# bbw7561135/Compton2d

Measured on AMD Instinct MI355X. Metric: photon-packet-steps/sec (whole node) at 1/2/4/8 GPUs; % HBM roofline, higher is better.
Workload: dtype f64

## Files before the change

compton2d_amd/csrc/c2d_device.hpp:

```cpp
#ifndef C2D_DEVICE_HPP
#define C2D_DEVICE_HPP

#include <stdint.h>
#include "../../include/compton2d.h"

namespace c2d {

#define C2D_IDX_BUCKETS 2048
struct Geo {
  double z[C2D_MAXZONE + 1];
  double r[C2D_MAXZONE + 1];
  double E_ph[C2D_N_VOL + 1];
  double E_field[C2D_NPHFIELD + 1];
  double hu[C2D_NPHOMAX + 2];
  double Elcmin[C2D_NPHLCMAX + 1];
  double Elcmax[C2D_NPHLCMAX + 1];
  double mu[C2D_NMUMAX + 1];
  int16_t eph_start[C2D_IDX_BUCKETS];
  int16_t efl_start[C2D_IDX_BUCKETS];
  int32_t eph_k0, efl_k0;
};
constexpr int GEO_DOUBLES = (int)(sizeof(Geo) / sizeof(double));

struct SpecDev {
// ... 40 lines not shown
  uint32_t sub;
};

struct PktSoA {
  double* rpre; double* zpre; double* wmu; double* phi; double* ew; double* xnu; double* dcen;
  uint32_t* jk;
  uint32_t* bins;
  uint32_t* ctr;
  uint32_t* sub;
  uint64_t* key;
};

struct TallyOff {
  int64_t edep, prdep, ecens, npcen, n_field, E_IC, nelectron, fout, edout;
  int64_t erlki, erlko, erlku, erlkl, Ed_in, counters;
};

#define C2D_EV_SHARDS 32
#ifndef C2D_TR_BLOCK
#define C2D_TR_BLOCK 256
#endif
#define C2D_EV_SHARD_STRIDE 16
#define C2D_EVQ_WORDS 8
#define C2D_EVQ_MAX 64
#define C2D_WORK_SHARDS 64

#ifndef C2D_COMTAB_N
#define C2D_COMTAB_N 2048
#endif
#define C2D_COMTAB_U0 (-27.631021115928547)
#define C2D_COMTAB_U1 (29.933606208922594)

__device__ __forceinline__ double c2d_tau_log_f32(double u) {
  const float v = (float)(1.0 - u);
  const float w = 1.0f - v;
  const bool lo = u < 0.5;
  const float lg = 0.69314718f * __builtin_amdgcn_logf(lo ? (float)u : w);
  const float r = (w == 1.0f) ? -v : lg * (v * __builtin_amdgcn_rcpf(1.0f - w));
  return (double)(lo ? lg : r);
}

enum : int32_t {
  ERR_CENSUS = 1, ERR_EVENT = 2, ERR_QUEUE = 4, ERR_SPEC = 8, ERR_NONFINITE = 16
};

#define C2D_GLOBAL __attribute__((address_space(1)))
template <class T>
__device__ __forceinline__ T gld(const T* p) { return *(const C2D_GLOBAL T*)p; }
template <class T>
__device__ __forceinline__ void gst(T* p, T v) { *(C2D_GLOBAL T*)p = v; }
__device__ __forceinline__ void cst2(c2d_d2* p, double a, double b) {
  const c2d_d2 v = {a, b};
  *(C2D_GLOBAL c2d_d2*)p = v;
}
__device__ __forceinline__ c2d_d2 cld2(const c2d_d2* p) { return *(const C2D_GLOBAL c2d_d2*)p; }
__device__ __forceinline__ void cst4(c2d_u4* p, uint32_t jk, uint32_t bins, uint64_t key) {
  const c2d_u4 v = {jk, bins, (uint32_t)key, (uint32_t)(key >> 32)};
  *(C2D_GLOBAL c2d_u4*)p = v;
}
__device__ __forceinline__ c2d_u4 cld4(const c2d_u4* p) { return *(const C2D_GLOBAL c2d_u4*)p; }
__device__ __forceinline__ uint64_t c2d_tg_key(c2d_u4 t) { return ((uint64_t)t.w << 32) | (uint64_t)t.z; }
__device__ __forceinline__ void cst2_nt(c2d_d2* p, double a, double b) {
  const c2d_d2 v = {a, b};
  __builtin_nontemporal_store(v, (C2D_GLOBAL c2d_d2*)p);
}
__device__ __forceinline__ c2d_d2 cld2_nt(const c2d_d2* p) {
  return __builtin_nontemporal_load((const C2D_GLOBAL c2d_d2*)p);
}
__device__ __forceinline__ void cst4_nt(c2d_u4* p, uint32_t jk, uint32_t bins, uint64_t key) {
  const c2d_u4 v = {jk, bins, (uint32_t)key, (uint32_t)(key >> 32)};
  __builtin_nontemporal_store(v, (C2D_GLOBAL c2d_u4*)p);
}
__device__ __forceinline__ c2d_u4 cld4_nt(const c2d_u4* p) {
  return __builtin_nontemporal_load((const C2D_GLOBAL c2d_u4*)p);
}
__device__ __forceinline__ uint32_t cens_bins(const c2d_u4* tg, int64_t s) {
  return gld(reinterpret_cast<const uint32_t*>(tg + s) + 1);
}
__device__ __forceinline__ void cens_set_bins(c2d_u4* tg, int64_t s, uint32_t b) {
  gst(reinterpret_cast<uint32_t*>(tg + s) + 1, b);
}
__device__ __forceinline__ void gadd(double* p, double v) {
  __hip_atomic_fetch_add((C2D_GLOBAL double*)p, v, __ATOMIC_RELAXED, __HIP_MEMORY_SCOPE_AGENT);
}

__device__ __forceinline__ void gor(int32_t* p, int32_t v) {
  __hip_atomic_fetch_or((C2D_GLOBAL int32_t*)p, v, __ATOMIC_RELAXED, __HIP_MEMORY_SCOPE_AGENT);
}

#ifndef C2D_NF_REPL
#define C2D_NF_REPL 8
#endif

#define C2D_CNT_PATHS_INT 10
#define C2D_CNT_DEAD_INT 12
#define C2D_CNT_CREUSE_INT 13
#define C2D_CNT_CLOST_INT 14

struct KParams {
  int32_t nz, nr, ncell, nphtotal, nph_lc, nmu;
  int32_t split1, split2, split3, spl3_trg, spec_switch;
  int32_t rank, world, ncycle, eps_linear;
  double time, dt, rmin, zmin, cdt;
  double cens_wlim;
  uint64_t step_key;
  const Geo* geo;
  const double* gnt;
  const double* kappa_cv;
  const double* kappa_s;
  const double* eps_tot;
  const double* eps_th;
  const double* f_nt;
  const double* Pnt;
  const double* n_e;
  const double* vfrac;
  const double* ewsv;
  const int64_t* vol_prefix;
  const int64_t* surf_prefix;
  const double* surf_ew;
  const double* surf_tbb;
  const int32_t* surf_spec;
  const double* tbbl;
  const SpecDev* spectra;
  int32_t n_spectra, nslot;
  const double* comtab;
  double comtab_du_inv;
  double egg_min;
  CensusSoA cin, cout;
  int64_t n_cin, cap_cout;
  uint32_t cens_chunk;
  unsigned long long* n_cout;
  const int32_t* clist;
  const int32_t* pool;
  const unsigned long long* pool_n;
  unsigned long long* pool_head;
  int32_t* out_list;
  unsigned long long* n_out;
  int32_t* relist;
  unsigned long long* n_relist;
  unsigned long long* relist_head;
  int64_t* cstate;
  double* ev;
  int64_t cap_ev;
  unsigned long long* n_ev_sh;
  int64_t cap_ev_sh;
  int64_t cap_q;
  PktSoA pk;
  int64_t cap_pk;
  int64_t n_cens_items, n_vol_items, n_surf_items;
  int64_t vol_cens_base;
  int64_t n_vol_global, n_surf_global;
  double* T;
  double* nf_rep;
  TallyOff off;
  unsigned long long* cnt;
  int32_t* err;
  int32_t lds_cells;
  int32_t evq_cap;
  unsigned long long* prof;
  const uint16_t* cdf_guide;
};
#define C2D_CDF_GUIDE 256

#define C2D_KN_CAP_DEFAULT 32
#define C2D_SC_K1_DEFAULT 16
struct GenArgs {
// ... 116 lines not shown
```

compton2d_amd/csrc/transport.hip:

```cpp
#include <hip/hip_runtime.h>

#ifndef C2D_FAST_MDIV
#define C2D_FAST_MDIV 1
#endif
#if defined(C2D_VARIANT) && C2D_VARIANT == 1 && C2D_FAST_MDIV
__device__ __forceinline__ double c2d_mdiv_rcp(double a, double b) {
  double y = __builtin_amdgcn_rcp(b);
  y = __builtin_fma(y, __builtin_fma(-b, y, 1.0), y);
  y = __builtin_fma(y, __builtin_fma(-b, y, 1.0), y);
  return a * y;
}
#define C2D_MDIV(a, b) c2d_mdiv_rcp((a), (b))
#endif
#ifndef C2D_FAST_FMA
#define C2D_FAST_FMA 0
#endif
#if defined(C2D_VARIANT) && C2D_VARIANT == 1 && C2D_FAST_FMA
#define C2D_MADD(a, b, c) __builtin_fma((a), (b), (c))
#endif

#include "c2d_device.hpp"
#include "c2d_math.h"
#include "c2d_rng.h"

// ... 617 lines not shown
  double gams = clampd(1.0 - (znue - znues) / (znu * znus), lim);
  for (;;) {
    if (++guard > 4 * MAX_REJECT) { CB_CNT(C2D_CNT_ABORTED); break; }
    wa = U(p);
    wb = 2.0 * U(p) - 1.0;
    swa = wa * wa + wb * wb;
    if (swa >= 1.0 || swa <= 1.0e-20) continue;
    break;
  }
  double cazs = clampd((wa * wa - wb * wb) / swa, lim);
  double wmus = p.wmu * gams +
                cazs * __builtin_sqrt((1.0 - gams * gams) * (1.0 - p.wmu * p.wmu + fuzz));
  wmus = clampd(wmus, lim);
  double xnus = znus * EMASSKEV;
  double cosdphi = clampd((gams - p.wmu * wmus) /
                              __builtin_sqrt((1.0 - p.wmu * p.wmu) * (1.0 - wmus * wmus)),
                          lim);
  double dphi = c2d_acos(cosdphi);
  double phis = p.phi + dphi;
  set_bins(p, bin_sp(g, P.nphtotal, xnus, 1.000001, 0.999999, 0), bin_lc(g, P.nph_lc, xnus),
           bin_mu(g, P.nmu, wmus));
  p.ew = p.ew * xnus / p.xnu;
  p.xnu = xnus;
  p.wmu = wmus;
  p.phi = phis;
  return st.i;
}

template <int TALLY = 1>
__device__ __forceinline__ int compb2d_w(const KParams& P, const Geo* g, double* nel, Pkt& p, bool run,
                                          int kn_cap) {
  KnState st;
  st.i = 0; st.j = 0; st.ctrA = 0;
  bool need = false;
  if (run) need = !kn_loop<TALLY>(P, nel, p, st, kn_cap < MAX_REJECT - 1 ? kn_cap : MAX_REJECT - 1);
  kn_coop<TALLY>(P, nel, p, st, need);
  int i_gam = 0;
  if (run) i_gam = compb2d_b<TALLY>(P, g, p, st);
  return i_gam;
}

__device__ __forceinline__ void push_event(const KParams& P0, double tb, const Pkt& p, LaneCnt& lc) {
  const KParams& P = cold(P0);
  const unsigned sh = blockIdx.x % C2D_EV_SHARDS;
  const unsigned long long slot = wave_reserve(P.n_ev_sh + sh * C2D_EV_SHARD_STRIDE);
  if (slot < (unsigned long long)P.cap_ev_sh) {
    double* e = P.ev + ((int64_t)sh * P.cap_ev_sh + (int64_t)slot) * C2D_EVENT_WORDS;
#if C2D_EV_NT
    EV_ST(e, tb); EV_ST(e + 1, p.xnu); EV_ST(e + 2, p.ew); EV_ST(e + 3, p.rpre); EV_ST(e + 4, p.zpre);
    EV_ST(e + 5, p.wmu); EV_ST(e + 6, p.phi);
#else
    gst(e, tb); gst(e + 1, p.xnu); gst(e + 2, p.ew); gst(e + 3, p.rpre); gst(e + 4, p.zpre);
    gst(e + 5, p.wmu); gst(e + 6, p.phi);
#endif
  } else {
    gor(P.err, ERR_EVENT);
  }
  LC_ADD(lc, C2D_CNT_EVENTS);
}

__device__ __forceinline__ void escape_tally(const KParams& P0, const Tal& T, const Pkt& p) {
  const KParams& P = cold(P0);
  const int32_t jgpsp = JGPSP(p), jgplc = JGPLC(p), jgpmu = JGPMU(p);
  if (jgplc > 0) atomicAdd(&T_EDOUT(P, T)[(jgpmu - 1) * C2D_NPHLCMAX + (jgplc - 1)], FDIV_POS(p.ew, P.dt));
  if (jgpsp > 0 && P.spec_switch == 0)
    atomicAdd(&T_FOUT(P, T)[(jgpmu - 1) * C2D_NPHOMAX + (jgpsp - 1)], p.ew);
}

C2D_COLD_FN int imcleak(const KParams& P0, const Tal& T, Pkt& p, LaneCnt& lc) {
  const KParams& P = cold(P0);
  if (p.kph == 0) {
    if (P.rmin > 1.0e-10) {
      atomicAdd(&T_ERLKI(P, T)[p.jph - 1], p.ew);
      LC_ADD(lc, C2D_CNT_ESCAPES);
      return 1;
    }
    p.phi = 1.0e-6;
    p.kph = 1;
    return 0;
  }
  LC_ADD(lc, C2D_CNT_ESCAPES);
  const double tb = P.time + P.dt - RAD_CP * p.dcen;
  if (p.jph <= 0) {
    if (P.tbbl[p.kph - 1] > 0.0) {
      gadd(&P.T[P.off.Ed_in + p.kph - 1], p.ew);
      atomicAdd(&T_ERLKL(P, T)[p.kph - 1], p.ew);
    }
    if (P.ncycle > 0) {
      push_event(P, tb, p, lc);
      escape_tally(P, T, p);
    }
    return 1;
  }
  if (p.jph != P.nz + 1) {
    atomicAdd(&T_ERLKO(P, T)[p.jph - 1], p.ew);
    if (P.ncycle > 0) {
      push_event(P, tb, p, lc);
      escape_tally(P, T, p);
    }
    return 1;
  }
  atomicAdd(&T_ERLKU(P, T)[p.kph - 1], p.ew);
  if (P.ncycle > 0 && p.wmu < F32(0.98)) {
    push_event(P, tb, p, lc);
    escape_tally(P, T, p);
  }
  return 1;
}

__device__ __forceinline__ int evq_offset(int evq_off) {
  return evq_off + __builtin_amdgcn_readfirstlane((int)((threadIdx.x >> 6) * C2D_EVQ_WORDS * C2D_EVQ_MAX));
}
__device__ __forceinline__ void evq_store(double* q, uint32_t i, const Pkt& p) {
  constexpr uint32_t cap = C2D_EVQ_MAX;
  q[i] = p.xnu;
  q[cap + i] = p.ew;
  q[2 * cap + i] = p.rpre;
  q[3 * cap + i] = p.zpre;
  q[4 * cap + i] = p.wmu;
#if C2D_TABLE_COMTOT
  q[5 * cap + i] = p.eta;
  const uint32_t sw = p.esw == -1 ? 0x80000000u : 0u;
#else
  q[5 * cap + i] = p.phi;
  const uint32_t sw = 0u;
#endif
  q[6 * cap + i] = p.dcen;
  const uint64_t tag = ((uint64_t)p.bins << 32) | (uint64_t)((uint32_t)p.kph | ((uint32_t)p.jph << 16) | sw);
  q[7 * cap + i] = __longlong_as_double((long long)tag);
}

__device__ __forceinline__ void evq_flush(const KParams& P0, const Tal& T, const double* q,
                                          uint32_t n, uint32_t lane, LaneCnt& lc) {
  constexpr uint32_t cap = C2D_EVQ_MAX;
  const KParams& P = cold(P0);
  if (lane >= n) return;
  Pkt p;
  p.xnu = q[lane];
  p.ew = q[cap + lane];
  p.rpre = q[2 * cap + lane];
  p.zpre = q[3 * cap + lane];
  p.wmu = q[4 * cap + lane];
  const double az = q[5 * cap + lane];
  p.dcen = q[6 * cap + lane];
  const uint64_t tag = (uint64_t)__double_as_longlong(q[7 * cap + lane]);
  p.bins = (uint32_t)(tag >> 32);
  p.kph = (int32_t)(tag & 0xffffu);
  p.jph = (int32_t)((tag >> 16) & 0x7fffu);
  LC_ADD(lc, C2D_CNT_ESCAPES);
  if (p.kph == 0) {
    atomicAdd(&T_ERLKI(P, T)[p.jph - 1], p.ew);
    return;
  }
  bool ev = P.ncycle > 0;
  if (p.jph <= 0) {
    if (P.tbbl[p.kph - 1] > 0.0) {
      gadd(&P.T[P.off.Ed_in + p.kph - 1], p.ew);
      atomicAdd(&T_ERLKL(P, T)[p.kph - 1], p.ew);
    }
  } else if (p.jph != P.nz + 1) {
    atomicAdd(&T_ERLKO(P, T)[p.jph - 1], p.ew);
  } else {
    atomicAdd(&T_ERLKU(P, T)[p.kph - 1], p.ew);
    ev = ev && p.wmu < F32(0.98);
  }
  if (!ev) return;
#if C2D_TABLE_COMTOT
  p.phi = c2d_acos(az);
  if (tag & 0x80000000ull) p.phi = 2.0 * PI_REF - p.phi;
#else
  p.phi = az;
#endif
  const double tb = P.time + P.dt - RAD_CP * p.dcen;
  push_event(P, tb, p, lc);
  escape_tally(P, T, p);
}

__shared__ unsigned long long c2d_cch_base[C2D_TR_BLOCK / 64];
__shared__ uint32_t c2d_cch_used[C2D_TR_BLOCK / 64];
__shared__ int32_t c2d_ct_idx[C2D_TR_BLOCK / 64][C2D_CT_TRACK];
__shared__ uint32_t c2d_ct_rem[C2D_TR_BLOCK / 64][C2D_CT_TRACK];
__shared__ int32_t c2d_fs[C2D_TR_BLOCK / 64][C2D_CT_STACK];
__shared__ uint32_t c2d_fs_n[C2D_TR_BLOCK / 64];
static_assert(C2D_WORK_CHUNK == C2D_CCHUNK, "a work chunk must cover exactly one census chunk");

C2D_COLD_FN unsigned long long census_new_chunk(const KParams& P0, int w) {
  const KParams& P = cold(P0);
  if (!P.clist)
    return __hip_atomic_fetch_add((C2D_GLOBAL unsigned long long*)P.n_cout, (unsigned long long)P.cens_chunk,
                                  __ATOMIC_RELAXED, __HIP_MEMORY_SCOPE_AGENT);
  int32_t id = -1;
  const uint32_t ns = c2d_fs_n[w];
  if (ns > 0) {
    id = c2d_fs[w][ns - 1];
    c2d_fs_n[w] = ns - 1;
  } else {
    if (__hip_atomic_load((C2D_GLOBAL unsigned long long*)P.n_relist, __ATOMIC_RELAXED,
                          __HIP_MEMORY_SCOPE_AGENT) > __hip_atomic_load((C2D_GLOBAL unsigned long long*)
                                                                          P.relist_head, __ATOMIC_RELAXED,
                                                                        __HIP_MEMORY_SCOPE_AGENT)) {
      const unsigned long long h = atomicAdd(P.relist_head, 1ull);
      if (h < gld(P.n_relist))
        id = __hip_atomic_load((C2D_GLOBAL int32_t*)(P.relist + h), __ATOMIC_RELAXED, __HIP_MEMORY_SCOPE_AGENT);
    }
    if (id < 0) {
      const unsigned long long h = atomicAdd(P.pool_head, 1ull);
      if (h < gld(P.pool_n)) id = gld(P.pool + h);
    }
  }
  if (id < 0) return (unsigned long long)P.cap_cout;
  gst(P.out_list + atomicAdd(P.n_out, 1ull), id);
  return (unsigned long long)id << C2D_CCHUNK_LOG;
}

__device__ __forceinline__ unsigned long long census_slot_chunk(const KParams& P0) {
  const KParams& P = cold(P0);
  const int w = (int)(threadIdx.x >> 6);
  const unsigned long long mask = __ballot(1);
  const uint32_t leader = (uint32_t)(__ffsll((long long)mask) - 1);
  const uint32_t lane = lane_id();
  const unsigned long long lt = (lane == 0) ? 0ull : (mask & ((~0ull) >> (64 - lane)));
  const uint32_t rank = (uint32_t)__popcll(lt), k = (uint32_t)__popcll(mask);
  const unsigned long long base = c2d_cch_base[w];
  const uint32_t used = c2d_cch_used[w];
  const uint32_t CENS_CHUNK = P.cens_chunk;
  const uint32_t rem = CENS_CHUNK - used;
  if (k <= rem) {
    if (lane == leader) c2d_cch_used[w] = used + k;
    return base + used + rank;
  }
  unsigned long long nb = 0;
  if (lane == leader) nb = census_new_chunk(P, w);
  const uint32_t lo = __builtin_amdgcn_readlane((uint32_t)nb, leader);
  const uint32_t hi = __builtin_amdgcn_readlane((uint32_t)(nb >> 32), leader);
  nb = ((unsigned long long)hi << 32) | lo;
  if (lane == leader) { c2d_cch_base[w] = nb; c2d_cch_used[w] = k - rem; }
  return rank < rem ? base + used + rank : nb + (rank - rem);
}

__device__ __forceinline__ void census_chunk_load(const KParams& P0, int w, uint32_t lane) {
  const KParams& P = cold(P0);
  if (lane != 0) return;
  c2d_cch_base[w] = 0ull;
  c2d_cch_used[w] = P.cens_chunk;
  c2d_fs_n[w] = 0u;
  for (int e = 0; e < C2D_CT_TRACK; e++) c2d_ct_idx[w][e] = -1;
  const int64_t ws = (int64_t)blockIdx.x * (C2D_TR_BLOCK / 64) + w;
  const int64_t base = gld(P.cstate + 2 * ws);
  if (base >= 0) {
    c2d_cch_base[w] = (unsigned long long)base;
    c2d_cch_used[w] = (uint32_t)gld(P.cstate + 2 * ws + 1);
  }
}

__device__ __forceinline__ void census_relist(const KParams& P, int32_t id) {
  const unsigned long long h = atomicAdd(P.n_relist, 1ull);
  __hip_atomic_store((C2D_GLOBAL int32_t*)(P.relist + h), id, __ATOMIC_RELAXED, __HIP_MEMORY_SCOPE_AGENT);
}

__device__ __forceinline__ void census_chunk_store(const KParams& P0, int w, uint32_t lane) {
  const KParams& P = cold(P0);
  if (lane != 0) return;
  if (P.clist)
    for (uint32_t i = 0; i < c2d_fs_n[w]; i++) census_relist(P, c2d_fs[w][i]);
  const uint32_t used = c2d_cch_used[w];
  const unsigned long long base = c2d_cch_base[w];
  const int64_t ws = (int64_t)blockIdx.x * (C2D_TR_BLOCK / 64) + w;
  const bool part = used < P.cens_chunk && base < (unsigned long long)P.cap_cout;
  gst(P.cstate + 2 * ws, part ? (int64_t)base : (int64_t)-1);
  gst(P.cstate + 2 * ws + 1, (int64_t)used);
}

__device__ __forceinline__ void census_track(int w, int32_t id, uint32_t n) {
#pragma unroll 1
  for (int k = 0; k < C2D_CT_TRACK; k++) {
    const int e = (id + k) & (C2D_CT_TRACK - 1);
    if (c2d_ct_idx[w][e] < 0) {
      c2d_ct_idx[w][e] = id;
      c2d_ct_rem[w][e] = n;
      return;
    }
  }
  atomicAdd(&c2d_cnt_lds[C2D_CNT_CLOST_INT], 1u);
}

C2D_COLD_FN void census_item_done(const KParams& P0, long long slot) {
  const KParams& P = cold(P0);
  const int w = (int)(threadIdx.x >> 6);
  const int32_t id = (int32_t)(slot >> C2D_CCHUNK_LOG);
  int e = id & (C2D_CT_TRACK - 1);
  if (c2d_ct_idx[w][e] != id) {
    int k = 1;
#pragma unroll 1
    for (; k < C2D_CT_TRACK; k++)
      if (c2d_ct_idx[w][(id + k) & (C2D_CT_TRACK - 1)] == id) break;
    if (k == C2D_CT_TRACK) return;
    e = (id + k) & (C2D_CT_TRACK - 1);
  }
  if (atomicSub(&c2d_ct_rem[w][e], 1u) != 1u) return;
  c2d_ct_idx[w][e] = -1;
  const uint32_t s = atomicAdd(&c2d_fs_n[w], 1u);
  if (s < C2D_CT_STACK) {
    c2d_fs[w][s] = id;
  } else {
    atomicSub(&c2d_fs_n[w], 1u);
    census_relist(P, id);
  }
  atomicAdd(&c2d_cnt_lds[C2D_CNT_CREUSE_INT], 1u);
}

C2D_COLD_FN void census_write(const KParams& P0, const Tal& T, const Pkt& p, LaneCnt& lc) {
  const KParams& P = cold(P0);
  const Geo* g = T.g;
  int cell = (p.jph - 1) * P.nr + (p.kph - 1);
  cell_add(P, T, TC_NPCEN, cell, 1.0);
  cell_add(P, T, TC_ECENS, cell, p.ew);
#if defined(C2D_ABLATE_NFIELD) && C2D_ABLATE_NFIELD == 1
  if (p.xnu < 0.0) {
#else
  int efl = 0;
  if (p.xnu > P.egg_min) {
#endif
    const int known = (p.ie >> 16) - 1;
    const int i = known >= 0 ? known : grid_lookup(g->E_field, C2D_NPHFIELD, g->efl_start, g->efl_k0, p.xnu);
    efl = i;
    const double v = FDIV_POS(6.25e8 * p.ew, p.xnu);
#if defined(C2D_ABLATE_NFIELD) && C2D_ABLATE_NFIELD == 2
    if (v == 1.25e300)
#endif
#if defined(C2D_ABLATE_NFIELD) && C2D_ABLATE_NFIELD == 3
    gst(&P.nf_rep[(int64_t)(blockIdx.x % C2D_NF_REPL) * P.ncell * C2D_NPHFIELD +
                  (int64_t)cell * C2D_NPHFIELD + (i - 1)], v);
    if (v == 1.25e300)
#endif
    gadd(&P.nf_rep[(int64_t)(blockIdx.x % C2D_NF_REPL) * P.ncell * C2D_NPHFIELD +
                   (int64_t)cell * C2D_NPHFIELD + (i - 1)], v);
  }
  const unsigned long long slot = census_slot_chunk(P);
  if (slot < (unsigned long long)P.cap_cout) {
// ... 86 lines not shown
  TP_POST = 5,
  TP_PTS = 6,
  TP_CWR = 7,
  TP_ITER = 8,
  TP_LANES = 9,
  TP_GOT_W = 10, TP_GOT_L = 11,
  TP_CENS_W = 12, TP_CENS_L = 13,
  TP_LEAK_W = 14, TP_LEAK_L = 15,
  TP_COLL_W = 16, TP_COLL_L = 17,
  TP_RST_W = 18, TP_RST_L = 19,
  TP_NWAVE = 20,
  TP_FLUSH = 21,
  TP_FLUSH_W = 22, TP_FLUSH_L = 23
};
enum : int { TP_CNT0 = TP_GOT_W, TP_CNT1 = TP_RST_L };
struct Prof {
#ifdef C2D_TR_PROF
  uint64_t acc[C2D_TR_PROF_WORDS];
  uint64_t t;
#endif
};
#ifdef C2D_TR_PROF
#define TP_MARK(pf, i) do { const uint64_t _n = clock64(); (pf).acc[i] += _n - (pf).t; (pf).t = _n; } while (0)
#define TP_COUNT(pf, iw, il) do {                                                         \
    const unsigned long long _m = __ballot(1);                                            \
    if (lane_id() == (uint32_t)(__ffsll((long long)_m) - 1)) {                            \
      (pf).acc[iw] += 1; (pf).acc[il] += __popcll(_m);                                    \
    }                                                                                     \
  } while (0)
#define TP_REPORT(pf, P, lane) do {                                                       \
    (pf).acc[TP_NWAVE] = 1;                                                               \
    for (int i = 0; i < C2D_TR_PROF_WORDS; i++)                                           \
      if ((pf).acc[i] && ((lane) == 0 || (i >= TP_CNT0 && i <= TP_CNT1)))                 \
        atomicAdd(&(P).prof[i], (unsigned long long)(pf).acc[i]);                         \
  } while (0)
#else
#define TP_MARK(pf, i) do { } while (0)
#define TP_COUNT(pf, iw, il) do { } while (0)
#endif

template <int V12>
__device__ __forceinline__ int flight(const KParams& P, const Tal& T, Pkt& p, ComCache& cc, LaneCnt& lc,
                                      Prof& pf) {
  const double lim8 = V12 ? 1.0 : 9.9999999e-1, lim9 = V12 ? 1.0 : 0.999999999;
  const Geo* g = T.g;
#if C2D_TABLE_COMTOT && C2D_EARLY_LOADS
  const int cell_e = (p.jph - 1) * P.nr + (p.kph - 1);
  const double* tb_e = P.comtab + (int64_t)cell_e * C2D_COMTAB_N + (p.tg > 0 ? p.tg - 1 : 0);
  const double ey0 = gld(tb_e), ey1 = gld(tb_e + 1), ey2 = gld(tb_e + 2), ey3 = gld(tb_e + 3);
  const double ene = gld(P.n_e + cell_e);
  const double ekap = gld((KAP(p) ? P.kappa_s : P.kappa_cv) + (int64_t)cell_e * C2D_N_VOL + ((p.ie & 0xffff) - 1));
#endif
  double colmfp = 0.0;
  if (p.mode != 0) colmfp = (V12 && p.nflight != 0) ? p.cmfp : -c2d_log(U(p));
  if (p.ew < 1.0e-40) return FL_END;
  if (++p.nflight > MAX_FLIGHTS) {
    LC_ADD(lc, C2D_CNT_ABORTED);
    return FL_END;
  }
  p.wmu = clampd(p.wmu, lim8);
  const int cell = (p.jph - 1) * P.nr + (p.kph - 1);
  double comac = 0.0;
  if (p.mode != 0) {
#if C2D_TABLE_COMTOT && C2D_EARLY_LOADS
    comac = (p.tg == 0) ? comtot_exact(P, cell, p.xnu)
                        : comtot_interp(ey0, ey1, ey2, ey3, ene, p.tt);
    (void)cc;
#elif C2D_TABLE_COMTOT
    comac = comtot_table(P, cell, p.xnu, p.tg, p.tt);
    (void)cc;
#else
    if (cc.cell0 == cell) {
      comac = cc.v0;
    } else if (cc.cell1 == cell) {
      comac = cc.v1;
    } else {
      comac = comtot_exact(P, cell, p.xnu);
      cc.cell1 = cc.cell0; cc.v1 = cc.v0;
      cc.cell0 = cell; cc.v0 = comac;
    }
#endif
  }
  const double sigsc = comac;
  const double rkm1 = (p.kph == 1) ? P.rmin : g->r[p.kph - 1];
  const double xqsqleft = rkm1 * rkm1;
  double dcol;
  if (p.mode != 0)
    dcol = colmfp / sigsc;
  else
    dcol = 100 * (g->r[P.nr] > g->z[P.nz] ? g->r[P.nr] : g->z[P.nz]);
  double trld;
  int ikind;
  if (p.dcen <= dcol) { trld = p.dcen; ikind = 2; }
  else { trld = dcol; ikind = 3; }
  lc.steps++;
#if C2D_TABLE_COMTOT
  double Eta = p.eta;
  const int eta_switch = p.esw;
#else
  double Eta = c2d_cos(p.phi);
  const int eta_switch = (p.phi <= PI_REF && p.phi >= 1.0e-10) ? 1 : -1;
#endif
  if (!V12) Eta = clampd(Eta, lim8);
  const double rpre = p.rpre, zpre = p.zpre, wmu = p.wmu;
  const double disp = Eta * rpre;
  const double psq = rpre * rpre * (1.0 - Eta * Eta);
  int kbnd, inout, knew, jnew;
  double rbnd, Zbnd;
  if (Eta < 0.0 && psq < xqsqleft) {
    kbnd = p.kph - 1;
    inout = -1;
    rbnd = rkm1;
  } else {
    kbnd = p.kph;
    inout = 1;
    rbnd = g->r[p.kph];
  }
  double dpbsq = rbnd * rbnd - psq;
  if (dpbsq < 1.0e-6) dpbsq = 1.0e-6;
  const double disbr = (double)inout * __builtin_sqrt(dpbsq) - disp;
  const double swmu = __builtin_sqrt(1.0 - wmu * wmu);
  double trldb = disbr / swmu;
  double fr = disbr;
  const double Zr = zpre + wmu * trldb;
  const double zlow = (p.jph == 1) ? P.zmin : g->z[p.jph - 1];
  const double zup = g->z[p.jph];
  if (Zr > zup || Zr < zlow) {
    Zbnd = (Zr > zup) ? zup : zlow;
    knew = p.kph;
    jnew = (Zr > zup) ? p.jph + 1 : p.jph - 1;
    const double f = (Zbnd - zpre) * swmu / wmu;
    fr = f;
    rbnd = __builtin_sqrt(rpre * rpre + f * f + 2.0 * rpre * f * Eta);
    trldb = __builtin_sqrt(f * f + (Zbnd - zpre) * (Zbnd - zpre));
  } else {
    knew = p.kph + inout;
    jnew = p.jph;
    rbnd = (kbnd > 0) ? g->r[kbnd] : P.rmin;
    Zbnd = Zr;
  }
  double rnew, znew;
  if (trldb < trld) {
    ikind = 1;
    trld = trldb;
    rnew = rbnd;
    znew = Zbnd;
  } else {
    jnew = p.jph;
    knew = p.kph;
    const double f = trld * swmu;
    fr = f;
    rnew = __builtin_sqrt(f * f + rpre * rpre + 2.0 * f * rpre * Eta);
    znew = zpre + trld * wmu;
  }
  TP_MARK(pf, TP_GEOM);
#if C2D_TABLE_COMTOT && C2D_EARLY_LOADS
  double sigabs = 1.0e-40 + 1.0 * ekap;
#else
  const double* kap = KAP(p) ? P.kappa_s : P.kappa_cv;
  double sigabs = 1.0e-40 + 1.0 * gld(kap + (int64_t)cell * C2D_N_VOL + ((p.ie & 0xffff) - 1));
#endif
  if (sigabs < 1.0e-40) sigabs = 1.0e-40;
  const double xabs = sigabs * trld;
  const double ewnew = (xabs < 100.0) ? p.ew * c2d_exp(-xabs) : 0.0;
  double deleabs = p.ew - ewnew;
  if (deleabs < 1.0e-50) deleabs = 1.0e-50;
  double wmustar;
  if (xabs <= 0.00001) {
    wmustar = wmu;
  } else {
    double mr, sstar = 0.0;
    for (int guard = 0; guard < MAX_REJECT; guard++) {
      mr = U(p);
      if (mr < p.ew / deleabs) {
        sstar = -c2d_log(1.0 - mr * deleabs / p.ew) / sigabs;
        break;
      }
    }
    const double denom = __builtin_sqrt(rpre * rpre + 2.0 * wmu * rpre * sstar + sstar * sstar);
    wmustar = (wmu * rpre + sstar) / denom;
  }
  const double delpr = deleabs * wmustar * C_LIGHT;
  if (p.mode != 0) {
    cell_add(P, T, TC_EDEP, cell, deleabs);
    cell_add(P, T, TC_PRDEP, cell, delpr);
  }
  TP_MARK(pf, TP_ABS);
  if (ewnew <= p.wtmin) {
    LC_ADD(lc, C2D_CNT_KILLED);
    return FL_END;
  }
  p.ew = ewnew;
  p.dcen = p.dcen - trld;
  if (V12)
    Eta = (fr + Eta * rpre) / rnew;
  else
    Eta = (trld + Eta * rpre) / rnew;
  Eta = clampd(Eta, lim9);
  if (V12 && ikind == 1) p.cmfp = colmfp - sigsc * trld;
  const bool leaves = (jnew == P.nz + 1 || jnew == 0 || knew == P.nr + 1 || knew == 0);
#if C2D_TABLE_COMTOT
  p.eta = Eta;
  if (p.mode != -1 && (ikind == 3 || leaves)) {
    p.phi = c2d_acos(Eta);
    if (eta_switch == -1) p.phi = 2.0 * PI_REF - p.phi;
  }
#else
  p.phi = c2d_acos(Eta);
  if (eta_switch == -1) p.phi = 2.0 * PI_REF - p.phi;
#endif
  p.rpre = rnew;
  p.zpre = znew;
  if (ikind == 1) {
    if (leaves) {
      p.jph = jnew;
      p.kph = knew;
      if (p.mode == -1) return FL_END;
      TP_COUNT(pf, TP_LEAK_W, TP_LEAK_L);
      if (imcleak(P, T, p, lc) == 1) {
        if (p.mode == 1) LC_ADD(lc, C2D_CNT_ESC_SCAT);
        return FL_END;
// ... 477 lines not shown
      if (pending) {
        i_gam = ig;
        if (it.is2 || p.ew > thr) { done = true; pending = false; }
        else if (k + 1u >= sc_k1) pending = false;
      }
    }
    if (!act) continue;
    if (it.is2 && p.ew > thr) {
      ScatRec r3 = it.rec;
      r3.key = p.key;
      r3.ctr = p.ctr;
      r3.sub = 0;
      push_scat(P, A.q3_out, A.n3_out, r3);
    } else if (done) {
      scat_emit(P, A, eic_lds, p, i_gam, ewold);
    } else {
      const unsigned long long h = wave_reserve(A.n_hard);
      if (h < (unsigned long long)P.cap_pk) A.hard[h] = item;
      else gor(P.err, ERR_QUEUE);
    }
  }
  __syncthreads();
  for (int i = threadIdx.x; i < C2D_NUM_NT + 2; i += SBLOCK) {
    if (nel_lds[i] != 0.0) atomicAdd(&P.T[P.off.nelectron + i], nel_lds[i]);
    if (eic_lds[i] != 0.0) atomicAdd(&P.T[P.off.E_IC + i], eic_lds[i]);
  }
  flush_counters(P, lc, lane_id());
}

__global__ void __launch_bounds__(SBLOCK) C2D_SFX(c2d_scatter_hard_kernel)(const KParams* __restrict__ Pg,
                                                                          const GenArgs A) {
  const KParams& P = *Pg;
  __shared__ double geo_lds[GEO_DOUBLES];
  __shared__ double nel_lds[C2D_NUM_NT + 2];
  __shared__ double eic_lds[C2D_NUM_NT + 2];
  for (int i = threadIdx.x; i < GEO_DOUBLES; i += SBLOCK)
    geo_lds[i] = reinterpret_cast<const double*>(P.geo)[i];
  for (int i = threadIdx.x; i < C2D_NUM_NT + 2; i += SBLOCK) {
    nel_lds[i] = 0.0;
    eic_lds[i] = 0.0;
  }
  init_counters(c2d_cnt_lds);
  __syncthreads();
  const Geo* g = reinterpret_cast<const Geo*>(geo_lds);
  LaneCnt lc = {0u};
  const uint32_t lane = lane_id();
  const int wpb = SBLOCK / 64;
  const int64_t n_hard = (int64_t)rfl64(*A.n_hard);
  const int64_t n_take = n_hard < P.cap_pk ? n_hard : P.cap_pk;
  for (int64_t h = (int64_t)blockIdx.x * wpb + (int64_t)(__builtin_amdgcn_readfirstlane(threadIdx.x) >> 6);
       h < n_take; h += (int64_t)gridDim.x * wpb) {
    const ScatItem it = scat_item(P, A, A.hard[h]);
    const double ewold = it.rec.ew / P.split2 / P.split3;
    const double thr = ewold * P.split2 * P.split1 * P.spl3_trg;
    const uint64_t key = c2d_derive_s(it.rec.key, C2D_TAG_SCAT3, it.ii, it.rec.ctr, it.rec.sub);
    for (uint32_t k0 = (uint32_t)A.sc_k1;; k0 += 64u) {
      const uint32_t k = k0 + lane;
      const bool live = k <= (uint32_t)MAX_REJECT;
      Pkt p;
      const int i_gam = scat_attempt(P, g, nel_lds, p, it.rec, key, k, ewold, live, A.kn_cap);
      const bool ok = live && (p.ew > thr || k == (uint32_t)MAX_REJECT);
      const unsigned long long m = __ballot(ok);
      if (m == 0ull) continue;
      const uint32_t kf = (uint32_t)(__ffsll((long long)m) - 1);
      {
        Pkt q;
        (void)scat_attempt<-1>(P, g, nel_lds, q, it.rec, key, k, ewold, live && lane > kf, A.kn_cap);
      }
      if (lane == kf) {
        if (!(p.ew > thr)) atomicAdd(&c2d_cnt_lds[C2D_CNT_ABORTED], 1u);
        scat_emit(P, A, eic_lds, p, i_gam, ewold);
      }
      break;
    }
  }
  __syncthreads();
  for (int i = threadIdx.x; i < C2D_NUM_NT + 2; i += SBLOCK) {
    if (nel_lds[i] != 0.0) atomicAdd(&P.T[P.off.nelectron + i], nel_lds[i]);
    if (eic_lds[i] != 0.0) atomicAdd(&P.T[P.off.E_IC + i], eic_lds[i]);
  }
  flush_counters(P, lc, lane_id());
}

struct CensRec {
  double rpre, zpre, wmu, cphi, ew, xnu;
  uint32_t jk, bn;
  uint64_t key;
};

__device__ __forceinline__ void pf_issue(const KParams& P0, CensRec& r, long long i) {
  const KParams& P = cold(P0);
  const c2d_d2 rz = CENS_LD2(P.cin.rz + i), wp = CENS_LD2(P.cin.wp + i), ex = CENS_LD2(P.cin.ex + i);
  const c2d_u4 tg = CENS_LD4(P.cin.tg + i);
  r.rpre = rz.x; r.zpre = rz.y;
  r.wmu = wp.x; r.cphi = wp.y;
  r.ew = ex.x; r.xnu = ex.y;
  r.jk = tg.x; r.bn = tg.y;
  r.key = c2d_tg_key(tg);
}

__device__ __forceinline__ void pf_apply(const KParams& P0, Pkt& p, const CensRec& r) {
  const KParams& P = cold(P0);
  p.rpre = r.rpre; p.zpre = r.zpre;
  p.wmu = clampd(r.wmu, P.cens_wlim);
  p.ew = r.ew; p.xnu = r.xnu;
#if C2D_TABLE_COMTOT
  p.eta = r.cphi;
  p.esw = (r.bn & C2D_CENS_ESW) ? -1 : 1;
  p.phi = 0.0;
#else
  p.phi = r.cphi;
#endif
  p.jph = c2d_cens_j(r.jk); p.kph = c2d_cens_k(r.jk);
  p.ie = c2d_cens_ie(r.jk) | ((c2d_cens_efl(r.jk) + 1) << 16);
  p.bins = r.bn & 0x00ffffffu;
  p.key = r.key;
  p.sub = 0;
  p.dcen = P.cdt;
  if (r.bn & C2D_CENS_VOL) p.dcen = P.cdt * c2d_draw_s(r.key, 0u, 0u);
}

#ifndef C2D_PF_LDS
#define C2D_PF_LDS 0
#endif
#if C2D_PF_LDS
__shared__ uint32_t c2d_pf_lds[C2D_TR_BLOCK / 64][16][64];
typedef const __attribute__((address_space(1))) void* c2d_gptr_t;
typedef __attribute__((address_space(3))) void* c2d_lptr_t;
__device__ __forceinline__ void pf_dword(const void* src, int w, int f) {
  __builtin_amdgcn_global_load_lds((c2d_gptr_t)src, (c2d_lptr_t)&c2d_pf_lds[w][f][0], 4, 0, 0);
}
__device__ __forceinline__ void pf_issue_lds(const KParams& P0, long long i) {
  const KParams& P = cold(P0);
  const int w = (int)(threadIdx.x >> 6);
  const uint32_t* d[4] = {reinterpret_cast<const uint32_t*>(P.cin.rz + i),
                          reinterpret_cast<const uint32_t*>(P.cin.wp + i),
                          reinterpret_cast<const uint32_t*>(P.cin.ex + i),
                          reinterpret_cast<const uint32_t*>(P.cin.tg + i)};
#pragma unroll
  for (int f = 0; f < 16; f++) pf_dword(d[f >> 2] + (f & 3), w, f);
}
__device__ __forceinline__ void pf_read_lds(CensRec& r) {
  __builtin_amdgcn_s_waitcnt(0xF70);
  const int w = (int)(threadIdx.x >> 6), l = (int)(threadIdx.x & 63);
  auto dbl = [&](int f) {
    return __hiloint2double((int)c2d_pf_lds[w][2 * f + 1][l], (int)c2d_pf_lds[w][2 * f][l]);
  };
  r.rpre = dbl(0); r.zpre = dbl(1); r.wmu = dbl(2); r.cphi = dbl(3); r.ew = dbl(4); r.xnu = dbl(5);
  r.jk = c2d_pf_lds[w][12][l];
  r.bn = c2d_pf_lds[w][13][l];
  r.key = ((uint64_t)c2d_pf_lds[w][15][l] << 32) | (uint64_t)c2d_pf_lds[w][14][l];
}
#endif

__device__ __forceinline__ void load_source(const KParams& P0, Pkt& p, long long src) {
  const KParams& P = cold(P0);
  if (src >= 0) {
    CensRec r;
    pf_issue(P, r, src);
    pf_apply(P, p, r);
  } else {
    load_pk(p, P.pk, -src - 1);
    set_phi(p, p.phi);
  }
}

template <int V12>
__global__ void __launch_bounds__(BLOCK) C2D_TR_ATTR C2D_SFX(c2d_transport_kernel)(const KParams* __restrict__ Pg,
                                                                      const GenArgs A) {
  const KParams& P = *Pg;
  double* const lds = c2d_tr_lds;
  const int tid = threadIdx.x;
  const uint32_t lane = lane_id();
  Tal T;
  T.g = reinterpret_cast<const Geo*>(lds);
  T.cells_off = GEO_DOUBLES;
  const int n_cells_lds = P.lds_cells ? 4 * P.ncell : 0;
  T.esc_off = GEO_DOUBLES + n_cells_lds;
  const int n_esc = P.nmu * (C2D_NPHOMAX + C2D_NPHLCMAX) + 2 * P.nz + 2 * P.nr;
  double* const cells_lds = lds + T.cells_off;
  double* const esc_lds = lds + T.esc_off;
  {
    const double* gsrc = reinterpret_cast<const double*>(P.geo);
    for (int i = tid; i < GEO_DOUBLES; i += BLOCK) lds[i] = gld(gsrc + i);
    for (int i = tid; i < n_cells_lds + n_esc; i += BLOCK) cells_lds[i] = 0.0;
  }
  init_counters(c2d_cnt_lds);
  census_chunk_load(P, tid >> 6, lane);
  __syncthreads();
  const long long n_items = (long long)rfl64(*A.n_pk);

  Pkt p;
  p.mode = 1; p.bins = 0u; p.ctr = 0; p.key = 0; p.sub = 0; p.nflight = 0;
  bool busy = false;
  ComCache cc = {-1, -1, 0.0, 0.0};
  LaneCnt lc = {0u};
  long long chunk_base = 0, chunk_end = 0;
  bool exhausted = false;
  Prof pf;
#ifdef C2D_TR_PROF
  for (int i = 0; i < C2D_TR_PROF_WORDS; i++) pf.acc[i] = 0;
  pf.t = clock64();
#endif

  for (;;) {
    bool got = false;
    long long item = -1;
    if (!exhausted) {
      unsigned long long needm = __ballot(!busy);
      while (needm != 0ull) {
        if (chunk_base >= chunk_end) {
          unsigned long long nb = 0;
          if (lane == 0) nb = atomicAdd(A.work_counter, (unsigned long long)CHUNK);
          nb = rfl64(nb);
          if ((long long)nb >= n_items) { exhausted = true; break; }
          chunk_base = (long long)nb;
          chunk_end = chunk_base + CHUNK < n_items ? chunk_base + CHUNK : n_items;
        }
        const long long avail = chunk_end - chunk_base;
        const unsigned long long lt = (lane == 0) ? 0ull : (needm & ((~0ull) >> (64 - lane)));
        const long long rank = __popcll(lt);
        const long long nneed = __popcll(needm);
        if (((needm >> lane) & 1ull) && rank < avail) {
          item = chunk_base + rank;
          got = true;
        }
// ... 138 lines not shown
  const double rnew = FSQRT(f * f + rpre * rpre + 2.0 * f * rpre * Eta);
  const double znew = zpre + trld * wmu;
  const double xabs = sigabs * trld;
  const double ewnew = (xabs < 100.0) ? b.ewp * FEXP(-xabs) : 0.0;
  double deleabs = b.ewp - ewnew;
  if (deleabs < 1.0e-50) deleabs = 1.0e-50;
  double wmustar;
  if (xabs <= 0.00001) {
    wmustar = wmu;
  } else {
    const double mr = UB(b);
    const double sstar = FDIV_POS(-FLOG(1.0 - FDIV_POS(mr * deleabs, b.ewp)), sigabs);
    const double denom = FSQRT(rpre * rpre + 2.0 * wmu * rpre * sstar + sstar * sstar);
    wmustar = FDIV_POS(wmu * rpre + sstar, denom);
  }
  cell_add(P, T, TC_EDEP, cell, deleabs);
  cell_add(P, T, TC_PRDEP, cell, deleabs * wmustar * C_LIGHT);
  if (ewnew <= b.wtminp) {
    LC_ADD(lc, C2D_CNT_KILLED);
    return;
  }
  LC_ADD(lc, C2D_CNT_COLLIDE);
  double Eta2 = clampd(FDIV_NN((V12 ? f : trld) + Eta * rpre, rnew), lim9);
  double phi = c2d_acos(Eta2);
  if (eta_switch == -1) phi = 2.0 * PI_REF - phi;
  ScatRec r;
  r.rpre = rnew; r.zpre = znew; r.wmu = wmu; r.phi = phi; r.ew = ewnew; r.xnu = p.xnu;
  r.dcen = p.dcen - trld;
  r.jk = ((uint32_t)p.jph << 16) | (uint32_t)p.kph;
  r.ctr = b.bctr;
  r.key = p.key;
  r.kap = (uint32_t)KAP(p);
  r.sub = 1u + (uint32_t)(b.g0 + i);
  push_scat(P, A.q2_out, A.n2_out, r);
  b.nscat++;
  if (b.flags & BF_SPEC) {
    lc.steps -= (uint32_t)b.tsteps;
    b.flags = (b.flags & ~(BF_TRACK | BF_SPEC | BF_TKILL | BF_TABORT)) | BF_RERUN;
  }
}

template <int V12, int EVQ>
__device__ __forceinline__ void bundle_step(const KParams& P1, const Tal& T, const GenArgs& A,
                                            Bundle& b, ComCache& cc, LaneCnt& lc, Prof& pf,
                                            CensRec& nr, long long nitem, int& nst) {
#ifdef C2D_HOT_RELOAD
  const KParams& P = cold_always(P1);
#else
  const KParams& P = P1;
#endif
  const double lim8 = V12 ? 1.0 : 9.9999999e-1, lim9 = V12 ? 1.0 : 0.999999999;
  const Geo* g = T.g;
  Pkt& p = b.p;
  if (b.alive && b.ewp < 1.0e-40) b.alive = 0;
  if ((b.flags & BF_TRACK) && p.ew < 1.0e-40) b.flags &= ~BF_TRACK;
  if (!b.alive && !(b.flags & BF_TRACK)) return;
  if (++p.nflight > MAX_FLIGHTS) {
    atomicAdd(&c2d_cnt_lds[C2D_CNT_ABORTED], (uint32_t)__popc(b.alive));
    b.alive = 0;
    if (b.flags & BF_TRACK) b.flags = (b.flags & ~BF_TRACK) | BF_TKILL | BF_TABORT;
    return;
  }
  p.wmu = clampd(p.wmu, lim8);
  lc.paths++;
  const int cell = (p.jph - 1) * P.nr + (p.kph - 1);
  const double kap_cell = gld((KAP(p) ? P.kappa_s : P.kappa_cv) + (int64_t)cell * C2D_N_VOL + ((p.ie & 0xffff) - 1));
  double sigsc = 1.0;
  if (b.alive) {
#if C2D_TABLE_COMTOT
    sigsc = comtot_table(P, cell, p.xnu, p.tg, p.tt);
    (void)cc;
#else
    if (cc.cell0 == cell) {
      sigsc = cc.v0;
    } else if (cc.cell1 == cell) {
      sigsc = cc.v1;
    } else {
      sigsc = comtot_exact(P, cell, p.xnu);
      cc.cell1 = cc.cell0; cc.v1 = cc.v0;
      cc.cell0 = cell; cc.v0 = sigsc;
    }
#endif
  }
  const double rkm1 = (p.kph == 1) ? P.rmin : g->r[p.kph - 1];
  const double xqsqleft = rkm1 * rkm1;
#if C2D_TABLE_COMTOT
  double Eta = p.eta;
  const int eta_switch = p.esw;
#else
  double Eta = c2d_cos(p.phi);
  const int eta_switch = (p.phi <= PI_REF && p.phi >= 1.0e-10) ? 1 : -1;
#endif
  if (!V12) Eta = clampd(Eta, lim8);
  const double rpre = p.rpre, zpre = p.zpre, wmu = p.wmu;
  const double disp = Eta * rpre;
  const double psq = rpre * rpre * (1.0 - Eta * Eta);
  int kbnd, inout, knew, jnew;
  double rbnd, Zbnd;
  if (Eta < 0.0 && psq < xqsqleft) {
    kbnd = p.kph - 1;
    inout = -1;
    rbnd = rkm1;
  } else {
    kbnd = p.kph;
    inout = 1;
    rbnd = g->r[p.kph];
  }
  double dpbsq = rbnd * rbnd - psq;
  if (dpbsq < 1.0e-6) dpbsq = 1.0e-6;
  const double disbr = (double)inout * FSQRT(dpbsq) - disp;
  const double swmu = FSQRT(1.0 - wmu * wmu);
  double trldb = FDIV_POS(disbr, swmu);
  double fr = disbr;
  const double Zr = zpre + wmu * trldb;
  const double zlow = (p.jph == 1) ? P.zmin : g->z[p.jph - 1];
  const double zup = g->z[p.jph];
  if (Zr > zup || Zr < zlow) {
    Zbnd = (Zr > zup) ? zup : zlow;
    knew = p.kph;
    jnew = (Zr > zup) ? p.jph + 1 : p.jph - 1;
    const double f = FDIV_POS((Zbnd - zpre) * swmu, wmu);
    fr = f;
    rbnd = FSQRT(rpre * rpre + f * f + 2.0 * rpre * f * Eta);
    trldb = FSQRT(f * f + (Zbnd - zpre) * (Zbnd - zpre));
  } else {
    knew = p.kph + inout;
    jnew = p.jph;
    rbnd = (kbnd > 0) ? g->r[kbnd] : P.rmin;
    Zbnd = Zr;
  }
  const bool bnd = trldb < p.dcen;
  const double trld = bnd ? trldb : p.dcen;
  double sigabs = 1.0e-40 + 1.0 * kap_cell;
  if (sigabs < 1.0e-40) sigabs = 1.0e-40;
  const double xabs = sigabs * trld;
  const double ex = (xabs < 100.0) ? FEXP(-xabs) : 0.0;
  const bool two = xabs > 0.00001;
  TP_MARK(pf, TP_GEOM);
  int nabs = 0;
  double dabs = 0.0, qabs = 0.0;
  if (b.alive) {
    int n = __popc(b.alive);
    lc.steps += (uint32_t)n;
    double dpos = 0.0;
    for (;;) {
      const double dcol = dpos + FDIV_POS(b.tau, sigsc);
      if (!(dcol < p.dcen && !(trldb < dcol))) break;
      int k = (int)(UB(b) * (double)n);
      if (k > n - 1) k = n - 1;
      uint32_t m = b.alive;
      for (; k > 0; k--) m &= m - 1u;
      const int i = __ffs(m) - 1;
      b.alive &= ~(1u << i);
      n--;
      probe_collide<V12>(P, T, A, b, i, dcol, sigabs, Eta, swmu, eta_switch, cell, lc);
      dpos = dcol;
      if (n == 0) break;
      b.tau = FDIV_POS(-TAU_LOG(UB(b)), (double)n);
    }
    if (n > 0) {
      b.tau = b.tau - sigsc * (trld - dpos);
      const double ewnew = (xabs < 100.0) ? b.ewp * ex : 0.0;
      double deleabs = b.ewp - ewnew;
      if (deleabs < 1.0e-50) deleabs = 1.0e-50;
      nabs = n;
      dabs = deleabs;
      qabs = FDIV_POS(deleabs, b.ewp);
      if (ewnew <= b.wtminp) {
        atomicAdd(&c2d_cnt_lds[C2D_CNT_KILLED], (uint32_t)n);
        b.alive = 0;
      } else {
        b.ewp = ewnew;
      }
    }
  }
  TP_MARK(pf, TP_ABS);
  if (b.flags & BF_TRACK) {
    lc.steps++;
    if (b.flags & BF_SPEC) b.tsteps++;
    const double ewnew = (xabs < 100.0) ? p.ew * ex : 0.0;
    if (two) p.ctr++;
    if (ewnew <= p.wtmin) b.flags = (b.flags & ~BF_TRACK) | BF_TKILL;
    else p.ew = ewnew;
  }
  if (b.alive || (b.flags & BF_TRACK)) {
    double rnew, znew;
    if (bnd) {
      rnew = rbnd;
      znew = Zbnd;
    } else {
      jnew = p.jph;
      knew = p.kph;
      const double f = trld * swmu;
      fr = f;
      rnew = FSQRT(f * f + rpre * rpre + 2.0 * f * rpre * Eta);
      znew = zpre + trld * wmu;
    }
    p.dcen = p.dcen - trld;
    double Etan = FDIV_NN((V12 ? fr : trld) + Eta * rpre, rnew);
    Etan = clampd(Etan, lim9);
    const bool leaves = bnd && (jnew == P.nz + 1 || jnew == 0 || knew == P.nr + 1 || knew == 0);
#if C2D_TABLE_COMTOT
    p.eta = Etan;
    if (!EVQ && (b.flags & BF_TRACK) && leaves) {
      p.phi = c2d_acos(Etan);
      if (eta_switch == -1) p.phi = 2.0 * PI_REF - p.phi;
    }
#else
    p.phi = c2d_acos(Etan);
    if (eta_switch == -1) p.phi = 2.0 * PI_REF - p.phi;
#endif
    p.rpre = rnew;
    p.zpre = znew;
    TP_MARK(pf, TP_EVENT);
    if (bnd) {
      if (leaves) {
        b.alive = 0;
        p.jph = jnew;
        p.kph = knew;
        if (b.flags & BF_TRACK) {
          TP_COUNT(pf, TP_LEAK_W, TP_LEAK_L);
          if (!EVQ) {
            if (imcleak(P, T, p, lc) == 1) b.flags &= ~BF_TRACK;
            else set_phi(p, p.phi);
          } else if (p.kph == 0 && !(P.rmin > 1.0e-10)) {
            p.kph = 1;
            set_phi(p, 1.0e-6);
          } else {
            b.flags = (b.flags & ~BF_TRACK) | BF_ESCQ;
          }
        }
      } else {
        p.kph = knew;
        p.jph = jnew;
      }
    } else {
      b.alive = 0;
      if (b.flags & BF_TRACK) {
        TP_COUNT(pf, TP_CENS_W, TP_CENS_L);
        census_write(P, T, p, lc);
        b.flags &= ~BF_TRACK;
      }
    }
    TP_MARK(pf, TP_CWR);
  }
  TP_MARK(pf, TP_EVENT);
#if C2D_PF_SRC
  if (nst == 1 && nitem >= 0) {
#if C2D_PF_LDS
    pf_issue_lds(P, nitem);
    (void)nr;
#else
    pf_issue(P, nr, nitem);
#endif
    nst = 2;
  }
#else
  (void)nr; (void)nitem; (void)nst;
#endif
  if (nabs > 0) {
    double sum_prdep = 0.0;
#ifdef C2D_ABLATE_PROBE_ABS
    if (two && nabs < 0) {
#else
    if (two) {
#endif
      const uint32_t sub = C2D_SUB_ABSPT | (uint32_t)b.g0;
#if C2D_TABLE_COMTOT && C2D_PT_F32
      {
        const double sr = sigabs * rpre;
        const double a = sr < 1.0 ? sr : 1.0;
        const float isig = (float)(sr > 1.0 ? FDIV_POS(1.0, sr) : 1.0);
        const float Aw = (float)(wmu * a);
        const float Cw = (float)(a * a * (1.0 - wmu * wmu));
        const float qf = (float)qabs;
        float wsum = 0.0f;
        uint64_t zst = p.key + 0x9E3779B97F4A7C15ull * ((((uint64_t)sub << 32) | (uint64_t)b.actr) + 1ull);
        for (int t = 0; t < nabs; t += 2) {
          const uint64_t wo = c2d_mix64(zst);
          zst += 0x9E3779B97F4A7C15ull;
          b.actr++;
#pragma unroll
          for (int j = 0; j < 2; j++) {
            if (t + j < nabs) {
              const uint32_t u = j == 0 ? (uint32_t)(wo >> 32) : (uint32_t)wo;
              float fu;
              __asm__("v_cvt_f32_u32 %0, %1" : "=v"(fu) : "v"(u >> 8));
              const float x = (fu + 0.5f) * (5.9604644775390625e-8f * qf);
              const float L = (x < 1.0e-2f)
                  ? x * __builtin_fmaf(x, __builtin_fmaf(x, __builtin_fmaf(x, 0.25f, 0.33333334f), 0.5f), 1.0f)
                  : -0.69314718f * __builtin_amdgcn_logf(1.0f - x);
              const float tt = __builtin_fmaf(L, isig, Aw);
              wsum += tt * __builtin_amdgcn_rsqf(__builtin_fmaf(tt, tt, Cw));
            }
          }
        }
        sum_prdep = dabs * (double)wsum * C_LIGHT;
      }
#else
// ... 413 lines not shown
```

Before: 275.3 billion.

## Simplify boundary lookups, use explicit global atomics, add vmcnt wait and branch hint

Several small edits. Generic atomicAdd calls on census list counters become explicit global relaxed agent-scope atomics, and tbbl reads go through gld. The rmin and zmin special cases in the transport step are dropped in favour of plain table reads, which assumes g->r[0]==rmin and g->z[0]==zmin, along with the redundant rbnd reassignment. A forced vmcnt(0) wait is inserted before the tracked-packet update and the leak branch is marked unlikely. The extra wait could stall on outstanding loads, and the geometry simplification is only correct if the tables hold those boundary values.

```diff
diff --git a/compton2d_amd/csrc/c2d_device.hpp b/compton2d_amd/csrc/c2d_device.hpp
--- a/compton2d_amd/csrc/c2d_device.hpp
+++ b/compton2d_amd/csrc/c2d_device.hpp
@@ -146,6 +146,10 @@
 }
 __device__ __forceinline__ void gadd(double* p, double v) {
   __hip_atomic_fetch_add((C2D_GLOBAL double*)p, v, __ATOMIC_RELAXED, __HIP_MEMORY_SCOPE_AGENT);
+}
+
+__device__ __forceinline__ unsigned long long gadd_u64(unsigned long long* p, unsigned long long v) {
+  return __hip_atomic_fetch_add((C2D_GLOBAL unsigned long long*)p, v, __ATOMIC_RELAXED, __HIP_MEMORY_SCOPE_AGENT);
 }
 
 __device__ __forceinline__ void gor(int32_t* p, int32_t v) {
diff --git a/compton2d_amd/csrc/transport.hip b/compton2d_amd/csrc/transport.hip
--- a/compton2d_amd/csrc/transport.hip
+++ b/compton2d_amd/csrc/transport.hip
@@ -723,7 +723,7 @@
   LC_ADD(lc, C2D_CNT_ESCAPES);
   const double tb = P.time + P.dt - RAD_CP * p.dcen;
   if (p.jph <= 0) {
-    if (P.tbbl[p.kph - 1] > 0.0) {
+    if (gld(P.tbbl + (p.kph - 1)) > 0.0) {
       gadd(&P.T[P.off.Ed_in + p.kph - 1], p.ew);
       atomicAdd(&T_ERLKL(P, T)[p.kph - 1], p.ew);
     }
@@ -795,7 +795,7 @@
   }
   bool ev = P.ncycle > 0;
   if (p.jph <= 0) {
-    if (P.tbbl[p.kph - 1] > 0.0) {
+    if (gld(P.tbbl + (p.kph - 1)) > 0.0) {
       gadd(&P.T[P.off.Ed_in + p.kph - 1], p.ew);
       atomicAdd(&T_ERLKL(P, T)[p.kph - 1], p.ew);
     }
@@ -840,17 +840,17 @@
                           __HIP_MEMORY_SCOPE_AGENT) > __hip_atomic_load((C2D_GLOBAL unsigned long long*)
                                                                           P.relist_head, __ATOMIC_RELAXED,
                                                                         __HIP_MEMORY_SCOPE_AGENT)) {
-      const unsigned long long h = atomicAdd(P.relist_head, 1ull);
+      const unsigned long long h = gadd_u64(P.relist_head, 1ull);
       if (h < gld(P.n_relist))
         id = __hip_atomic_load((C2D_GLOBAL int32_t*)(P.relist + h), __ATOMIC_RELAXED, __HIP_MEMORY_SCOPE_AGENT);
     }
     if (id < 0) {
-      const unsigned long long h = atomicAdd(P.pool_head, 1ull);
+      const unsigned long long h = gadd_u64(P.pool_head, 1ull);
       if (h < gld(P.pool_n)) id = gld(P.pool + h);
     }
   }
   if (id < 0) return (unsigned long long)P.cap_cout;
-  gst(P.out_list + atomicAdd(P.n_out, 1ull), id);
+  gst(P.out_list + gadd_u64(P.n_out, 1ull), id);
   return (unsigned long long)id << C2D_CCHUNK_LOG;
 }
 
@@ -895,7 +895,7 @@
 }
 
 __device__ __forceinline__ void census_relist(const KParams& P, int32_t id) {
-  const unsigned long long h = atomicAdd(P.n_relist, 1ull);
+  const unsigned long long h = gadd_u64(P.n_relist, 1ull);
   __hip_atomic_store((C2D_GLOBAL int32_t*)(P.relist + h), id, __ATOMIC_RELAXED, __HIP_MEMORY_SCOPE_AGENT);
 }
 
@@ -1148,7 +1148,7 @@
 #endif
   }
   const double sigsc = comac;
-  const double rkm1 = (p.kph == 1) ? P.rmin : g->r[p.kph - 1];
+  const double rkm1 = g->r[p.kph - 1];
   const double xqsqleft = rkm1 * rkm1;
   double dcol;
   if (p.mode != 0)
@@ -1171,14 +1171,12 @@
   const double rpre = p.rpre, zpre = p.zpre, wmu = p.wmu;
   const double disp = Eta * rpre;
   const double psq = rpre * rpre * (1.0 - Eta * Eta);
-  int kbnd, inout, knew, jnew;
+  int inout, knew, jnew;
   double rbnd, Zbnd;
   if (Eta < 0.0 && psq < xqsqleft) {
-    kbnd = p.kph - 1;
     inout = -1;
     rbnd = rkm1;
   } else {
-    kbnd = p.kph;
     inout = 1;
     rbnd = g->r[p.kph];
   }
@@ -1189,7 +1187,7 @@
   double trldb = disbr / swmu;
   double fr = disbr;
   const double Zr = zpre + wmu * trldb;
-  const double zlow = (p.jph == 1) ? P.zmin : g->z[p.jph - 1];
+  const double zlow = g->z[p.jph - 1];
   const double zup = g->z[p.jph];
   if (Zr > zup || Zr < zlow) {
     Zbnd = (Zr > zup) ? zup : zlow;
@@ -1202,7 +1200,6 @@
   } else {
     knew = p.kph + inout;
     jnew = p.jph;
-    rbnd = (kbnd > 0) ? g->r[kbnd] : P.rmin;
     Zbnd = Zr;
   }
   double rnew, znew;
@@ -1846,6 +1843,8 @@
   flush_counters(P, lc, lane_id());
 }
 
+constexpr int C2D_WAIT_VMCNT0 = 0x0F70;
+
 struct CensRec {
   double rpre, zpre, wmu, cphi, ew, xnu;
   uint32_t jk, bn;
@@ -1905,7 +1904,7 @@
   for (int f = 0; f < 16; f++) pf_dword(d[f >> 2] + (f & 3), w, f);
 }
 __device__ __forceinline__ void pf_read_lds(CensRec& r) {
-  __builtin_amdgcn_s_waitcnt(0xF70);
+  __builtin_amdgcn_s_waitcnt(C2D_WAIT_VMCNT0);
   const int w = (int)(threadIdx.x >> 6), l = (int)(threadIdx.x & 63);
   auto dbl = [&](int f) {
     return __hiloint2double((int)c2d_pf_lds[w][2 * f + 1][l], (int)c2d_pf_lds[w][2 * f][l]);
@@ -2210,7 +2209,7 @@
     }
 #endif
   }
-  const double rkm1 = (p.kph == 1) ? P.rmin : g->r[p.kph - 1];
+  const double rkm1 = g->r[p.kph - 1];
   const double xqsqleft = rkm1 * rkm1;
 #if C2D_TABLE_COMTOT
   double Eta = p.eta;
@@ -2223,14 +2222,12 @@
   const double rpre = p.rpre, zpre = p.zpre, wmu = p.wmu;
   const double disp = Eta * rpre;
   const double psq = rpre * rpre * (1.0 - Eta * Eta);
-  int kbnd, inout, knew, jnew;
+  int inout, knew, jnew;
   double rbnd, Zbnd;
   if (Eta < 0.0 && psq < xqsqleft) {
-    kbnd = p.kph - 1;
     inout = -1;
     rbnd = rkm1;
   } else {
-    kbnd = p.kph;
     inout = 1;
     rbnd = g->r[p.kph];
   }
@@ -2241,7 +2238,7 @@
   double trldb = FDIV_POS(disbr, swmu);
   double fr = disbr;
   const double Zr = zpre + wmu * trldb;
-  const double zlow = (p.jph == 1) ? P.zmin : g->z[p.jph - 1];
+  const double zlow = g->z[p.jph - 1];
   const double zup = g->z[p.jph];
   if (Zr > zup || Zr < zlow) {
     Zbnd = (Zr > zup) ? zup : zlow;
@@ -2254,7 +2251,6 @@
   } else {
     knew = p.kph + inout;
     jnew = p.jph;
-    rbnd = (kbnd > 0) ? g->r[kbnd] : P.rmin;
     Zbnd = Zr;
   }
   const bool bnd = trldb < p.dcen;
@@ -2303,6 +2299,7 @@
     }
   }
   TP_MARK(pf, TP_ABS);
+  __builtin_amdgcn_s_waitcnt(C2D_WAIT_VMCNT0);
   if (b.flags & BF_TRACK) {
     lc.steps++;
     if (b.flags & BF_SPEC) b.tsteps++;
@@ -2342,7 +2339,7 @@
     p.zpre = znew;
     TP_MARK(pf, TP_EVENT);
     if (bnd) {
-      if (leaves) {
+      if (__builtin_expect(leaves, 0)) {
         b.alive = 0;
         p.jph = jnew;
         p.kph = knew;
```

After: 292.5 billion, median of 6. 6.3% higher.
